# samiazirar/mvtracker

Hardware: AMD Instinct MI355X
Metric: query-points*frames/sec, 4-view 24-frame 512x512 @1024 queries (higher is better)
Workload: dtype bf16; 1 GPU; c3: 4-view synthetic 24-frame 512x512, 1024 queries, bf16 (configs[2], the metric's config); 4-view 24-frame 512x512, 1024 queries per GPU, corr K=16 x 4 levels, iters=4, 3 windows, random-init weights (seeded recipe); queries_total=1024, parallelism=query-shard x1, frame_store=bf16 rows

## Files before the change

### mvtracker_amd/csrc/block_fused.hip

```cpp
#include "common.h"
#include <stdlib.h>

namespace {

typedef __bf16 bf16x8 __attribute__((ext_vector_type(8)));
typedef __bf16 bf16x4 __attribute__((ext_vector_type(4)));
typedef unsigned u32x4 __attribute__((ext_vector_type(4)));
typedef unsigned u32x2 __attribute__((ext_vector_type(2)));

__device__ __forceinline__ void lds_barrier() {
#ifdef MVT_FULL_BARRIERS
  __syncthreads();
#else
  __builtin_amdgcn_fence(__ATOMIC_RELEASE, "workgroup", "local");
  __builtin_amdgcn_s_barrier();
  __builtin_amdgcn_fence(__ATOMIC_ACQUIRE, "workgroup", "local");
#endif
}

constexpr int NT = 512;
constexpr int C = 256;
constexpr int LDX = C + 8;
template <int NMB> struct Cfg {
  static constexpr int BM = 32 * NMB;
// ... 278 lines not shown
                                             int vstride = 0) {
  const int r = lane & 31, h = lane >> 5;
  const float scale = 1.0f / sqrtf((float)DHA);
  auto stage_vt = [&](int kb, unsigned short* img) {
    const int key = kb * 32 + r;
#pragma unroll
    for (int i = 0; i < 6; ++i) {
      u32x2 w = f.v[kb][i];
      if (key >= nk) w = (u32x2){0u, 0u};
#pragma unroll
      for (int e = 0; e < 4; ++e) img[(24 * h + 4 * i + e) * LDVA + r] = (unsigned short)((e & 1) ? (w[e >> 1] >> 16) : (w[e >> 1] & 0xFFFFu));
    }
  };
  if (vstride > 0) {
    __builtin_amdgcn_fence(__ATOMIC_SEQ_CST, "wavefront");
#pragma unroll
    for (int kb = 0; kb < NKB; ++kb) stage_vt(kb, vt + kb * vstride);
    __builtin_amdgcn_fence(__ATOMIC_SEQ_CST, "wavefront");
  }
  __builtin_amdgcn_sched_barrier(0);
  ASTAMP(49);
  bf16x8 qf[NMBQ][3];
#pragma unroll
  for (int mb = 0; mb < NMBQ; ++mb) {
#pragma unroll
    for (int ks = 0; ks < 3; ++ks) {
      f32x4 a = bf4_to_f32(f.q[mb][ks][0], f.q[mb][ks][1]), b = bf4_to_f32(f.q[mb][ks][2], f.q[mb][ks][3]);
#pragma unroll
      for (int e = 0; e < 4; ++e) {
        a[e] *= scale;
        b[e] *= scale;
      }
      const bf16x4 x = __builtin_convertvector(a, bf16x4), y = __builtin_convertvector(b, bf16x4);
#pragma unroll
      for (int e = 0; e < 4; ++e) {
        qf[mb][ks][e] = x[e];
        qf[mb][ks][4 + e] = y[e];
      }
    }
  }
  const unsigned bdm = bd > 0 ? (65536u / (unsigned)bd + 1u) : 0u;
#pragma unroll
  for (int mb = 0; mb < NMBQ; ++mb) {
    const int qi = mb * 32 + r;
    const unsigned qt = ((unsigned)qi * bdm) >> 16;
    f32x16 sc[NKB];
    float mx = -INFINITY;
#pragma unroll
    for (int kb = 0; kb < NKB; ++kb) {
#pragma unroll
      for (int e = 0; e < 16; ++e) sc[kb][e] = 0.f;
#pragma unroll
      for (int ks = 0; ks < 3; ++ks) sc[kb] = __builtin_amdgcn_mfma_f32_32x32x16_bf16(__builtin_bit_cast(bf16x8, f.k[kb][ks]), qf[mb][ks], sc[kb], 0, 0, 0);
    }
#pragma unroll
    for (int kb = 0; kb < NKB; ++kb) {
      const bool half = nk <= kb * 32 + 16;
#pragma unroll
      for (int e = 0; e < 16; ++e) {
        const unsigned kk = (unsigned)(kb * 32 + (e & 3) + 8 * (e >> 2)) + 4u * (unsigned)h;
        const bool ok = (kk < (unsigned)nk) & (((kk * bdm) >> 16) == qt);
        sc[kb][e] = ok ? sc[kb][e] : -INFINITY;
      }
#pragma unroll
      for (int e = 0; e < 8; ++e) mx = fmaxf(mx, sc[kb][e]);
      if (!half) {
#pragma unroll
        for (int e = 8; e < 16; ++e) mx = fmaxf(mx, sc[kb][e]);
      }
    }
    mx = pair_max(mx);
    if (mx == -INFINITY) mx = 0.f;
    float ps = 0.f;
#pragma unroll
    for (int kb = 0; kb < NKB; ++kb) {
      const bool half = nk <= kb * 32 + 16;
#pragma unroll
      for (int e = 0; e < 8; ++e) {
        sc[kb][e] = __expf(sc[kb][e] - mx);
        ps += sc[kb][e];
      }
      if (!half) {
#pragma unroll
        for (int e = 8; e < 16; ++e) {
          sc[kb][e] = __expf(sc[kb][e] - mx);
          ps += sc[kb][e];
        }
      }
    }
    __builtin_amdgcn_sched_barrier(0);
    ASTAMP(50 + 2 * mb);
    f32x16 oacc[2];
#pragma unroll
    for (int db = 0; db < 2; ++db)
#pragma unroll
      for (int e = 0; e < 16; ++e) oacc[db][e] = 0.f;
#pragma unroll
    for (int kb = 0; kb < NKB; ++kb) {
      const bool half = nk <= kb * 32 + 16;
      const unsigned short* vimg = vt + kb * vstride;
      if (vstride == 0 && (mb == 0 || NKB > 1)) {
        __builtin_amdgcn_fence(__ATOMIC_SEQ_CST, "wavefront");
        stage_vt(kb, vt);
        __builtin_amdgcn_fence(__ATOMIC_SEQ_CST, "wavefront");
      }
#pragma unroll
      for (int sk = 0; sk < 2; ++sk) {
        if (sk == 1 && half) break;
        f32x4 lo4, hi4;
#pragma unroll
        for (int e = 0; e < 4; ++e) {
          lo4[e] = sc[kb][8 * sk + e];
          hi4[e] = sc[kb][8 * sk + 4 + e];
        }
        const bf16x4 bl = __builtin_convertvector(lo4, bf16x4), bh = __builtin_convertvector(hi4, bf16x4);
        bf16x8 pb;
#pragma unroll
        for (int e = 0; e < 4; ++e) {
          pb[e] = bl[e];
          pb[4 + e] = bh[e];
        }
#pragma unroll
        for (int db = 0; db < 2; ++db) {
          const unsigned short* vr = (db * 32 + r < DHA) ? &vimg[(db * 32 + r) * LDVA + 16 * sk + 4 * h] : zrow + 16 * sk + 4 * h;
          const u32x2 a0 = *reinterpret_cast<const u32x2*>(vr), a1 = *reinterpret_cast<const u32x2*>(vr + 8);
          const bf16x8 va = __builtin_bit_cast(bf16x8, (u32x4){a0[0], a0[1], a1[0], a1[1]});
          oacc[db] = __builtin_amdgcn_mfma_f32_32x32x16_bf16(va, pb, oacc[db], 0, 0, 0);
        }
      }
    }
    __builtin_amdgcn_sched_barrier(0);
    ASTAMP(51 + 2 * mb);
    const float lt = pair_sum(ps);
    const float inv = 1.0f / lt;
    if (qi >= nq) continue;
#pragma unroll
    for (int db = 0; db < 2; ++db) {
#pragma unroll
      for (int gq = 0; gq < 4; ++gq) {
        const int d = db * 32 + 8 * gq + 4 * h;
        if (d < DHA) {
          f32x4 t;
#pragma unroll
          for (int e = 0; e < 4; ++e) t[e] = oacc[db][4 * gq + e] * inv;
          *reinterpret_cast<u32x2*>(&As[(arow0 + qi) * lda + hd * DHA + d]) = __builtin_bit_cast(u32x2, __builtin_convertvector(t, bf16x4));
        }
      }
    }
  }
}

template <int NMB>
__device__ __forceinline__ void ln_to_lds(const f32x16 (&v)[NMB], unsigned short* Xs, float* st, int wave, int lane, float eps,
                                          const float* lnw, const float* lnb, float (&ms)[NMB][2], bool have) {
  constexpr int BM = 32 * NMB;
  const int r = lane & 31, h = lane >> 5;
  f32x4 gw[4], gb[4];
  if (lnw) {
#pragma unroll
    for (int g = 0; g < 4; ++g) {
      gw[g] = *reinterpret_cast<const f32x4*>(lnw + wave * 32 + 8 * g + 4 * h);
      gb[g] = *reinterpret_cast<const f32x4*>(lnb + wave * 32 + 8 * g + 4 * h);
    }
  }
  if (!have) {
#pragma unroll
    for (int mb = 0; mb < NMB; ++mb) {
      float s1 = 0.f, s2 = 0.f;
#pragma unroll
      for (int e = 0; e < 16; ++e) {
        s1 += v[mb][e];
        s2 = fmaf(v[mb][e], v[mb][e], s2);
      }
      s1 += __shfl_xor(s1, 32, 64);
      s2 += __shfl_xor(s2, 32, 64);
      if (h == 0) {
        st[(wave * BM + mb * 32 + r) * 2] = s1;
        st[(wave * BM + mb * 32 + r) * 2 + 1] = s2;
      }
    }
    lds_barrier();
#pragma unroll
    for (int mb = 0; mb < NMB; ++mb) {
      float s1 = 0.f, s2 = 0.f;
#pragma unroll
      for (int w = 0; w < 8; ++w) {
        s1 += st[(w * BM + mb * 32 + r) * 2];
        s2 += st[(w * BM + mb * 32 + r) * 2 + 1];
      }
      const float mean = s1 / (float)C;
      ms[mb][0] = mean;
      ms[mb][1] = fmaxf(s2 / (float)C - mean * mean, 0.f);
    }
  }
#pragma unroll
  for (int mb = 0; mb < NMB; ++mb) {
    const float mean = ms[mb][0];
    const float rstd = 1.0f / sqrtf(ms[mb][1] + eps);
#pragma unroll
    for (int g = 0; g < 4; ++g) {
      const int n = wave * 32 + 8 * g + 4 * h;
      f32x4 o;
#pragma unroll
      for (int e = 0; e < 4; ++e) {
        o[e] = (v[mb][4 * g + e] - mean) * rstd;
        if (lnw) o[e] = o[e] * gw[g][e] + gb[g][e];
      }
      const bf16x4 b = __builtin_convertvector(o, bf16x4);
      *reinterpret_cast<u32x2*>(&Xs[(mb * 32 + r) * LDX + n]) = __builtin_bit_cast(u32x2, b);
    }
  }
  lds_barrier();
}

template <int NMB, int MODE, int ATT>
__global__ __launch_bounds__(NT) void block_fused_bf16(BlockArgs p) {
  using K_ = Cfg<NMB>;
  constexpr int BM = K_::BM, HC = K_::HC, LDH = K_::LDH, LDA = K_::LDA;
  constexpr bool CTX = ATT == 6;
  static_assert(!CTX || (NMB == 2 && MODE == 0), "ATT 6 runs on the 64-row tiles of the point rows");
  constexpr int HSZ = CTX && (64 * LDKV + 1) / 2 > BM * LDH ? (64 * LDKV + 1) / 2 : BM * LDH;
  __shared__ __attribute__((aligned(16))) unsigned short Xs[BM * LDX];
  __shared__ __attribute__((aligned(16))) unsigned short Hs[2][HSZ];
  __shared__ float st[8 * BM * 2];
  __shared__ __attribute__((aligned(16))) float b1s[4 * C];
  __shared__ __attribute__((aligned(16))) float cbs[CTX ? 2 * 288 : 4];

  const int t = threadIdx.x, wave = t >> 6, lane = t & 63;
  const int r = lane & 31, h = lane >> 5;
  int bx = (int)blockIdx.x, by = (int)blockIdx.y, bz = (int)blockIdx.z;
  if constexpr (ATT == 2 || ATT == 3 || ATT == 5 || ATT == 6) {
    const unsigned total = gridDim.x * gridDim.y * gridDim.z;
    if (total % 8 == 0) {
      const unsigned L = blockIdx.x + gridDim.x * (blockIdx.y + gridDim.y * blockIdx.z);
      const unsigned V = (L % 8) * (total / 8) + L / 8;
      bx = (int)(V % gridDim.x);
      by = (int)((V / gridDim.x) % gridDim.y);
      bz = (int)(V / (gridDim.x * gridDim.y));
    }
  }
  static_assert(ATT == 0 || ATT == 5 || MODE != 2, "pass 2 of the split path has no attention");
  static_assert(ATT != 5 || MODE == 2, "ATT 5 = pass 2 on the frame-major tiles of an ATT 2 / ATT 3 pass 1");
  static_assert((MODE != 1 && MODE != 2) || NMB == 1, "the split path runs on 32-row tiles");
  constexpr bool FM = ATT == 2 || ATT == 3 || ATT == 5 || ATT == 6;
  const int bmv = ATT == 1 ? p.bmv : BM;
  const long long m0 = FM ? 0 : (long long)bx * bmv;
  const long long ntok = FM ? p.M / p.S : 0;
  auto grow = [&](int i) -> long long {
    if (FM) {
      const long long tk = (long long)bx * BM + i;
      return tk < ntok ? tk * p.S + (long long)bz : -1;
    }
    const long long m = m0 + i;
    return (i < bmv && m < p.M) ? m : -1;
  };
  const long long rlo = FM ? (long long)bx * BM * p.S : m0;
  const long long rhi = FM ? ((long long)bx * BM + BM) * p.S : m0 + bmv;
  constexpr bool HAS_MLP = MODE == 0 || MODE == 1;
  if (HAS_MLP)
    for (int i = t; i < p.H; i += NT) b1s[i] = p.b1[i];
  const long long ws_tile = FM ? (long long)bz * gridDim.x + bx : (long long)bx;
  const long long ws_ntile = FM ? (long long)gridDim.z * gridDim.x : (long long)gridDim.x;
  auto ws_off = [&](int chunk, int g) -> long long { return ((((long long)chunk * ws_ntile + ws_tile) * 8 + wave) * 4 + g) * 256 + lane * 4; };
  auto active = [&](int q) { return q < p.n_next && rlo < p.next[q].row_hi && rhi > p.next[q].row_lo; };
  bf16x8 wq[PFQ];
  constexpr bool EARLY = NMB == 1 && MODE != 0;
  bool early_have = false;
  const bool outp = MODE != 2 && ATT != 4 && (ATT != 0 || p.att != nullptr);
  const unsigned short* wo_row = p.wo + ((long long)wave * 18 * 64 + lane) * 8;
  const unsigned short* fc1_first = p.w1 + ((long long)(wave % K_::JW) * (C / 16) * 64 + lane) * 8 +
                                    (long long)(MODE == 1 ? by : 0) * K_::JW * (C / 16) * FS;
  auto prefetch_wo = [&]() { fill_wq(wq, wo_row); };
  if (HAS_MLP && !outp) {
    fill_wq(wq, fc1_first);
  } else if (CTX) {
    fill_wq(wq, p.c_kv.w + ((long long)wave * (C / 16) * 64 + lane) * 8);
  } else if (outp) {
    prefetch_wo();
  } else if (EARLY && MODE == 2) {
    const int nb0e = by * 8 + wave;
    if (active(0) && nb0e < (p.next[0].N + 31) / 32) {
      fill_wq(wq, p.next[0].w + ((long long)nb0e * (C / 16) * 64 + lane) * 8);
      early_have = true;
    }
  }

  STAMP(0);
  f32x16 v[NMB];
#pragma unroll
  for (int mb = 0; mb < NMB; ++mb)
#pragma unroll
    for (int e = 0; e < 16; ++e) v[mb][e] = 0.f;

  f32x4 xr[NMB][4];
  auto load_x = [&]() {
    if (ATT == 4 || (MODE == 2 && p.ws)) return;
#pragma unroll
    for (int mb = 0; mb < NMB; ++mb) {
      const long long m = grow(mb * 32 + r);
#pragma unroll
      for (int g = 0; g < 4; ++g)
        xr[mb][g] = m >= 0 ? *reinterpret_cast<const f32x4*>(p.x + m * (long long)p.ldx + wave * 32 + 8 * g + 4 * h) : (f32x4){0.f, 0.f, 0.f, 0.f};
    }
  };

  bf16x8 wx[2];
  auto pre_gemm = [&]() {
    wx[0] = ldg_frag(wo_row + 16 * FS);
    wx[1] = ldg_frag(wo_row + 17 * FS);
    load_x();
  };

  if constexpr (CTX) {
    constexpr int KVB = 2 * 288 / 32;
    unsigned short* KV = &Hs[0][0];
    unsigned short* XN = &Xs[0];
    for (int i = t; i < KVB * 32; i += NT) cbs[i] = p.c_kv.b[i];
    const long long ctile = 2LL * gridDim.z;
    auto cws_off = [&](int chunk, int mb, int g) -> long long {
      return ((((long long)chunk * ctile + (long long)bz * 2 + mb) * 8 + wave) * 4 + g) * 256 + lane * 4;
    };
    constexpr int MAXCH = 4;
    const int nch = p.c_nch;
    f32x16 cv[2];
#pragma unroll
    for (int gh = 0; gh < 2; ++gh) {
      f32x4 part[2][2][MAXCH + 1], b2v[2];
#pragma unroll
      for (int mb = 0; mb < 2; ++mb)
#pragma unroll
        for (int g = 0; g < 2; ++g)
#pragma unroll
          for (int sidx = 0; sidx <= MAXCH; ++sidx)
            part[mb][g][sidx] = sidx <= nch ? *reinterpret_cast<const f32x4*>(p.c_ws + cws_off(sidx, mb, 2 * gh + g)) : (f32x4){0.f, 0.f, 0.f, 0.f};
#pragma unroll
      for (int g = 0; g < 2; ++g) b2v[g] = *reinterpret_cast<const f32x4*>(p.c_b2 + wave * 32 + 8 * (2 * gh + g) + 4 * h);
      __builtin_amdgcn_sched_barrier(0);
#pragma unroll
      for (int mb = 0; mb < 2; ++mb)
#pragma unroll
        for (int g = 0; g < 2; ++g) {
          f32x4 xv = part[mb][g][0];
#pragma unroll
          for (int sidx = 1; sidx <= MAXCH; ++sidx)
            if (sidx <= nch) {
#pragma unroll
              for (int e = 0; e < 4; ++e) xv[e] += part[mb][g][sidx][e];
            }
#pragma unroll
          for (int e = 0; e < 4; ++e) cv[mb][4 * (2 * gh + g) + e] = 0.f + (xv[e] + b2v[g][e]);
        }
      __builtin_amdgcn_sched_barrier(0);
    }
    STAMP(56);
    auto krow_w = [&](int nb) { return p.c_kv.w + ((long long)nb * (C / 16) * 64 + lane) * 8; };
    auto nrow_w = [&](int nb) { return p.c_next.w + ((long long)nb * (C / 16) * 64 + lane) * 8; };
    if (bx == 0) {
#pragma unroll
      for (int mb = 0; mb < 2; ++mb) {
        const long long m = (long long)(mb * 32 + r) * p.S + (long long)bz;
#pragma unroll
        for (int g = 0; g < 4; ++g) {
          f32x4 o;
#pragma unroll
          for (int e = 0; e < 4; ++e) o[e] = cv[mb][4 * g + e];
          *reinterpret_cast<f32x4*>(p.c_x + m * (long long)p.c_ldx + wave * 32 + 8 * g + 4 * h) = o;
        }
      }
    }
    float cms[2][2];
    ln_to_lds<2>(cv, XN, st, wave, lane, p.c_kv.eps, p.c_kv.lnw, p.c_kv.lnb, cms, false);
    STAMP(57);
    const int nnb = p.c_next.w ? (p.c_next.N + 31) / 32 : 0;
    const bool do_next = bx * 8 < nnb;
    const int nbn = bx * 8 + wave;
    const bool my_next = nbn < nnb;
#pragma unroll 1
    for (int nb = wave; nb < KVB; nb += 8) {
// ... 278 lines not shown
    STAMP(2);
    lds_barrier();
    STAMP(3);
    gemm_wq18<NMB, HAS_MLP>(v, wq, wx, fc1_first, &As[r * LDA + 8 * h], LDA);
#pragma unroll
    for (int mb = 0; mb < NMB; ++mb)
#pragma unroll
      for (int e = 0; e < 16; ++e) v[mb][e] += p.bo[wave * 32 + (e & 3) + 8 * (e >> 2) + 4 * h];
  } else {
    load_x();
  }
  STAMP(4);
  if (MODE == 2 && p.ws) {
    constexpr int MAXCH = 4;
    const int nch = p.H / Cfg<NMB>::HC;
    f32x4 part[NMB][4][MAXCH + 1];
#pragma unroll
    for (int mb = 0; mb < NMB; ++mb) {
      const long long m = grow(mb * 32 + r);
#pragma unroll
      for (int g = 0; g < 4; ++g)
#pragma unroll
        for (int sidx = 0; sidx <= MAXCH; ++sidx)
          part[mb][g][sidx] = (m >= 0 && sidx <= nch) ? *reinterpret_cast<const f32x4*>(p.ws + ws_off(sidx, g)) : (f32x4){0.f, 0.f, 0.f, 0.f};
    }
    __builtin_amdgcn_sched_barrier(0);
#pragma unroll
    for (int mb = 0; mb < NMB; ++mb)
#pragma unroll
      for (int g = 0; g < 4; ++g) {
        f32x4 xv = part[mb][g][0];
#pragma unroll
        for (int sidx = 1; sidx <= MAXCH; ++sidx)
          if (sidx <= nch) {
#pragma unroll
            for (int e = 0; e < 4; ++e) xv[e] += part[mb][g][sidx][e];
          }
#pragma unroll
        for (int e = 0; e < 4; ++e) v[mb][4 * g + e] += xv[e] + p.b2[wave * 32 + 8 * g + 4 * h + e];
      }
  } else if (ATT != 4) {
#pragma unroll
    for (int mb = 0; mb < NMB; ++mb)
#pragma unroll
      for (int g = 0; g < 4; ++g)
#pragma unroll
        for (int e = 0; e < 4; ++e) v[mb][4 * g + e] += xr[mb][g][e];
  }

  auto store_x = [&]() {
#pragma unroll
    for (int mb = 0; mb < NMB; ++mb) {
      const long long m = grow(mb * 32 + r);
      if (m >= 0) {
#pragma unroll
        for (int g = 0; g < 4; ++g) {
          f32x4 o;
#pragma unroll
          for (int e = 0; e < 4; ++e) o[e] = v[mb][4 * g + e];
          *reinterpret_cast<f32x4*>(p.x + m * (long long)p.ldx + wave * 32 + 8 * g + 4 * h) = o;
        }
      }
    }
  };
  STAMP(5);
  float ln_ms[NMB][2];
  if (HAS_MLP) ln_to_lds<NMB>(v, Xs, st, wave, lane, 1e-6f, nullptr, nullptr, ln_ms, false);
  STAMP(6);
  const bool tail_next = MODE == 0 && active(0) && wave < (p.next[0].N + 31) / 32;
  if (HAS_MLP) {
    f32x16 acc2[NMB];
#pragma unroll
    for (int mb = 0; mb < NMB; ++mb)
#pragma unroll
      for (int e = 0; e < 16; ++e) acc2[mb][e] = 0.f;
    constexpr int JW = K_::JW, NM1 = K_::NM1;
    const int jb = wave % JW, mp = wave / JW;
    const int nchunk = p.H / HC;
    const unsigned short* w1row = p.w1 + ((long long)jb * (C / 16) * 64 + lane) * 8;
    const unsigned short* w2row = p.w2 + ((long long)wave * (p.H / 16) * 64 + lane) * 8;
    static_assert(HC / 16 == PFQ && C / 16 == PFQ, "every GEMM segment is exactly one queue length");
    const unsigned short* tail = tail_next ? p.next[0].w + ((long long)wave * (C / 16) * 64 + lane) * 8 : w1row;
    const int c_lo = MODE == 1 ? by : 0, c_hi = MODE == 1 ? c_lo + 1 : nchunk;
#pragma unroll 1
    for (int c = c_lo; c < c_hi; ++c) {
      unsigned short* Hb = Hs[c & 1];
      f32x16 ha[NM1];
#pragma unroll
      for (int i = 0; i < NM1; ++i)
#pragma unroll
        for (int e = 0; e < 16; ++e) ha[i][e] = 0.f;
      STAMP(8 + 5 * c);
      gemm_wq<C / 16, NM1>(ha, wq, w1row + (long long)c * JW * (C / 16) * FS, w2row + (long long)c * (HC / 16) * FS, &Xs[r * LDX + 8 * h], LDX,
                           NM1 * mp);
      STAMP(9 + 5 * c);
#pragma unroll
      for (int i = 0; i < NM1; ++i) {
#pragma unroll
        for (int g = 0; g < 4; ++g) {
          const f32x4 bq = *reinterpret_cast<const f32x4*>(&b1s[c * HC + jb * 32 + 8 * g + 4 * h]);
          f32x4 o;
#ifdef MVT_ABL_NOGELU
#pragma unroll
          for (int e = 0; e < 4; ++e) o[e] = ha[i][4 * g + e] + bq[e];
#else
#pragma unroll
          for (int e = 0; e < 4; e += 2) {
            const f32x2 y = gelu_tanh_pk((f32x2){ha[i][4 * g + e] + bq[e], ha[i][4 * g + e + 1] + bq[e + 1]});
            o[e] = y[0];
            o[e + 1] = y[1];
          }
#endif
          const bf16x4 b = __builtin_convertvector(o, bf16x4);
          *reinterpret_cast<u32x2*>(&Hb[((NM1 * mp + i) * 32 + r) * LDH + jb * 32 + 8 * g + 4 * h]) = __builtin_bit_cast(u32x2, b);
        }
      }
      STAMP(10 + 5 * c);
      lds_barrier();
      STAMP(11 + 5 * c);
      const unsigned short* after = c + 1 < c_hi ? w1row + (long long)(c + 1) * JW * (C / 16) * FS : tail;
      gemm_wq<HC / 16, NMB>(acc2, wq, w2row + (long long)c * (HC / 16) * FS, after, &Hb[r * LDH + 8 * h], LDH, 0);
      STAMP(12 + 5 * c);
    }
    if (MODE == 1) {
#pragma unroll
      for (int mb = 0; mb < NMB; ++mb) {
        const long long m = grow(mb * 32 + r);
        if (m < 0) continue;
#pragma unroll
        for (int g = 0; g < 4; ++g) {
          f32x4 a4, x4;
#pragma unroll
          for (int e = 0; e < 4; ++e) {
            a4[e] = acc2[mb][4 * g + e];
            x4[e] = v[mb][4 * g + e];
          }
          *reinterpret_cast<f32x4*>(p.ws + ws_off(by + 1, g)) = a4;
          if (by == 0) *reinterpret_cast<f32x4*>(p.ws + ws_off(0, g)) = x4;
        }
      }
      return;
    }
#pragma unroll
    for (int mb = 0; mb < NMB; ++mb)
#pragma unroll
      for (int g = 0; g < 4; ++g)
#pragma unroll
        for (int e = 0; e < 4; ++e) v[mb][4 * g + e] += acc2[mb][4 * g + e] + p.b2[wave * 32 + 8 * g + 4 * h + e];
  }
  STAMP(30);
  if (MODE == 0 || ATT == 4 || (p.ws && by == 0)) store_x();
  STAMP(31);

  bool have = tail_next || early_have;
  bool have_ms = false;
#pragma unroll
  for (int q = 0; q < MVT_BLOCK_MAX_NEXT; ++q) {
    if (q >= p.n_next) break;
    if (!active(q)) continue;
    const mvt_block_next nx = p.next[q];
    lds_barrier();
    for (int i = t; i < nx.N; i += NT) b1s[i] = nx.b[i];
    STAMP(32 + 8 * q);
    ln_to_lds<NMB>(v, Xs, st, wave, lane, nx.eps, nx.lnw, nx.lnb, ln_ms, have_ms);
    have_ms = true;
    STAMP(33 + 8 * q);
    const int nblocks = (nx.N + 31) / 32;
    auto nrow_of = [&](int nb) { return nx.w + ((long long)nb * (C / 16) * 64 + lane) * 8; };
    const int nb0 = MODE == 2 ? by * 8 + wave : wave, nbstep = MODE == 2 ? 8 * (int)gridDim.y : 8;
    if (nb0 < nblocks && !have) fill_wq(wq, nrow_of(nb0));
    const int qn = q + 1 < MVT_BLOCK_MAX_NEXT ? q + 1 : MVT_BLOCK_MAX_NEXT - 1;
    const unsigned short* chain = nullptr;
    if ((MODE == 0 || MODE == 3) && q + 1 < MVT_BLOCK_MAX_NEXT && active(q + 1) && wave < (p.next[qn].N + 31) / 32)
      chain = p.next[qn].w + ((long long)wave * (C / 16) * 64 + lane) * 8;
    have = chain != nullptr && wave < nblocks;
    for (int nb = nb0; nb < nblocks; nb += nbstep) {
      f32x16 acc[NMB];
#pragma unroll
      for (int mb = 0; mb < NMB; ++mb)
#pragma unroll
        for (int e = 0; e < 16; ++e) acc[mb][e] = 0.f;
      gemm_wq<C / 16, NMB>(acc, wq, nrow_of(nb), nb + nbstep < nblocks ? nrow_of(nb + nbstep) : (chain ? chain : nrow_of(nb)), &Xs[r * LDX + 8 * h], LDX, 0);
      STAMP(34 + 8 * q + (nb - nb0) / nbstep);
      if (nx.y_bf16 && nb * 32 + 31 < nx.N && (nx.ldy & 7) == 0 && ((uintptr_t)nx.y & 15) == 0) {
        unsigned short* tile = &Hs[0][0] + wave * (NMB * 32 * YLD);
        __builtin_amdgcn_fence(__ATOMIC_SEQ_CST, "wavefront");
#pragma unroll
        for (int mb = 0; mb < NMB; ++mb)
#pragma unroll
          for (int g = 0; g < 4; ++g) {
            f32x4 o;
#pragma unroll
            for (int e = 0; e < 4; ++e) o[e] = acc[mb][4 * g + e] + b1s[nb * 32 + 8 * g + 4 * h + e];
            *reinterpret_cast<u32x2*>(&tile[(mb * 32 + r) * YLD + 8 * g + 4 * h]) = __builtin_bit_cast(u32x2, __builtin_convertvector(o, bf16x4));
          }
        __builtin_amdgcn_fence(__ATOMIC_SEQ_CST, "wavefront");
        unsigned short* yb = reinterpret_cast<unsigned short*>(nx.y) + nb * 32;
#pragma unroll
        for (int k = 0; k < NMB * 2; ++k) {
          const int pc = lane + 64 * k, row = pc >> 2, c = pc & 3;
          const long long m = grow(row);
          if (m >= nx.row_lo && m < nx.row_hi)
            *reinterpret_cast<u32x4*>(yb + m * (long long)nx.ldy + c * 8) = *reinterpret_cast<const u32x4*>(&tile[row * YLD + c * 8]);
        }
        continue;
      }
#pragma unroll
      for (int mb = 0; mb < NMB; ++mb) {
        const long long m = grow(mb * 32 + r);
        if (m < nx.row_lo || m >= nx.row_hi) continue;
#pragma unroll
        for (int g = 0; g < 4; ++g) {
          const int n = nb * 32 + 8 * g + 4 * h;
          if (n + 3 < nx.N) {
            f32x4 o;
#pragma unroll
            for (int e = 0; e < 4; ++e) o[e] = acc[mb][4 * g + e] + b1s[n + e];
            store_act4(nx.y, m * (long long)nx.ldy + n, o, nx.y_bf16);
          } else {
#pragma unroll
            for (int e = 0; e < 4; ++e)
              if (n + e < nx.N) store_act(nx.y, m * (long long)nx.ldy + n + e, acc[mb][4 * g + e] + b1s[n + e], nx.y_bf16);
          }
        }
      }
    }
    STAMP(39 + 8 * q);
  }
  STAMP(63);
}

__global__ void pack_frag_kernel(const unsigned short* __restrict__ w, int ld, int N, int K, unsigned short* __restrict__ out) {
  const long long total = (long long)((N + 31) / 32) * (K / 16) * 64;
  for (long long i = blockIdx.x * (long long)blockDim.x + threadIdx.x; i < total; i += (long long)gridDim.x * blockDim.x) {
    const int lane = (int)(i & 63);
    const long long f = i >> 6;
    const int ks = (int)(f % (K / 16));
    const int nb = (int)(f / (K / 16));
    const int n = nb * 32 + (lane & 31), k = ks * 16 + 8 * (lane >> 5);
    u32x4 v = (u32x4){0u, 0u, 0u, 0u};
    if (n < N) v = *reinterpret_cast<const u32x4*>(w + (long long)n * ld + k);
    *reinterpret_cast<u32x4*>(out + i * 8) = v;
  }
}

}

#ifdef MVT_STAMPS
extern "C" int mvt_debug_read_stamps(unsigned long long* host) {
  return hipMemcpyFromSymbol(host, HIP_SYMBOL(mvt_stamp_buf), sizeof(unsigned long long) * 2 * 8 * 64) == hipSuccess ? MVT_OK : MVT_ERR_HIP_BASE;
}
extern "C" int mvt_debug_clear_stamps() {
  static unsigned long long z[2 * 8 * 64];
  return hipMemcpyToSymbol(HIP_SYMBOL(mvt_stamp_buf), z, sizeof(z)) == hipSuccess ? MVT_OK : MVT_ERR_HIP_BASE;
}
#endif

extern "C" int mvt_pack_frag_bf16(const unsigned short* w, int ld, int N, int K, unsigned short* out, void* stream) {
  MVT_REQUIRE(w && out && N > 0 && K > 0 && K % 16 == 0 && ld % 8 == 0 && ld >= K);
  MVT_REQUIRE(((uintptr_t)w % 16 == 0) && ((uintptr_t)out % 16 == 0));
  const long long total = (long long)((N + 31) / 32) * (K / 16) * 64;
  hipLaunchKernelGGL(pack_frag_kernel, dim3((unsigned)mvt_cdiv(total, 256)), dim3(256), 0, mvt_stream(stream), w, ld, N, K, out);
  return mvt_launch_status();
}

extern "C" int mvt_block_fused_bf16(float* x, int ldx, const void* att, int att_bf16, int ldatt, int Ko, const unsigned short* wo, int ldwo,
                                    const float* bo, const unsigned short* w1, int ldw1, const float* b1, const unsigned short* w2,
                                    int ldw2, const float* b2, int H, const mvt_block_next* next, int n_next, long long M, int Cc,
                                    float* workspace, void* stream) {
  MVT_REQUIRE(x && w1 && b1 && w2 && b2 && M > 0 && Cc == C && H > 0 && H % 256 == 0 && H <= 4 * C);
  MVT_REQUIRE(ldx % 4 == 0 && ldx >= C);
  MVT_REQUIRE(!att || (wo && bo && Ko == 288 && ldatt % 4 == 0 && ldatt >= Ko));
  MVT_REQUIRE(n_next >= 0 && n_next <= MVT_BLOCK_MAX_NEXT && (n_next == 0 || next));
  MVT_REQUIRE(((uintptr_t)x % 16 == 0) && ((uintptr_t)att % 16 == 0) && ((uintptr_t)wo % 16 == 0) && ((uintptr_t)w1 % 16 == 0) &&
              ((uintptr_t)w2 % 16 == 0));
  BlockArgs a{};
  a.x = x; a.ldx = ldx; a.att = (const float*)att; a.att_bf16 = att_bf16 ? 1 : 0; a.ldatt = ldatt; a.Ko = Ko; a.wo = wo; a.bo = bo; a.ldwo = ldwo;
  a.w1 = w1; a.b1 = b1; a.w2 = w2; a.b2 = b2; a.ldw1 = ldw1; a.ldw2 = ldw2; a.H = H; a.M = M; a.n_next = n_next;
  for (int q = 0; q < n_next; ++q) {
    const mvt_block_next& nx = next[q];
    MVT_REQUIRE(nx.w && nx.b && nx.y && nx.N > 0 && nx.N <= 4 * C && nx.ldy % 4 == 0 && nx.ldy >= nx.N);
    MVT_REQUIRE(nx.y_bf16 == 0 || nx.y_bf16 == 1);
    MVT_REQUIRE((nx.lnw == nullptr) == (nx.lnb == nullptr) && ((uintptr_t)nx.lnw % 16 == 0) && ((uintptr_t)nx.lnb % 16 == 0) && ((uintptr_t)nx.w % 16 == 0) && ((uintptr_t)nx.y % 16 == 0));
    MVT_REQUIRE(nx.row_lo >= 0 && (nx.row_hi == 0 || nx.row_hi > nx.row_lo));
    a.next[q] = nx;
    if (nx.row_hi == 0) a.next[q].row_hi = M;
  }
  static const char* force = getenv("MVT_BLOCK_NMB");
  const int nmb = force ? atoi(force) : (M >= 4096 ? 2 : 1);
  static const bool no_split = getenv("MVT_BLOCK_NOSPLIT") != nullptr;
  a.ws = workspace;
  if (nmb == 2) {
    hipLaunchKernelGGL((block_fused_bf16<2, 0, 0>), dim3((unsigned)mvt_cdiv(M, 64)), dim3(NT), 0, mvt_stream(stream), a);
  } else if (workspace && !no_split && M <= 2048 && M % 32 == 0) {
    MVT_REQUIRE((uintptr_t)workspace % 16 == 0);
    const unsigned tiles = (unsigned)mvt_cdiv(M, 32);
    hipLaunchKernelGGL((block_fused_bf16<1, 1, 0>), dim3(tiles, (unsigned)(H / 256)), dim3(NT), 0, mvt_stream(stream), a);
    int maxblk = 1;
    for (int q = 0; q < n_next; ++q) maxblk = (next[q].N + 31) / 32 > maxblk ? (next[q].N + 31) / 32 : maxblk;
    const unsigned slices = n_next ? (unsigned)mvt_cdiv(maxblk, 8) : 1u;
    hipLaunchKernelGGL((block_fused_bf16<1, 2, 0>), dim3(tiles, slices), dim3(NT), 0, mvt_stream(stream), a);
  } else {
    hipLaunchKernelGGL((block_fused_bf16<1, 0, 0>), dim3((unsigned)mvt_cdiv(M, 32)), dim3(NT), 0, mvt_stream(stream), a);
  }
  return mvt_launch_status();
}

extern "C" int mvt_attn_block_fused_bf16(float* x, int ldx, const mvt_block_attn* attn, const unsigned short* wo, const float* bo,
                                         const unsigned short* w1, const float* b1, const unsigned short* w2, const float* b2, int H,
                                         const mvt_block_next* next, int n_next, long long M, int Cc, float* workspace, void* stream) {
  MVT_REQUIRE(x && attn && wo && bo && w1 && b1 && w2 && b2 && M > 0 && Cc == C && H > 0 && H % 256 == 0 && H <= 4 * C);
  MVT_REQUIRE(ldx % 4 == 0 && ldx >= C && n_next >= 0 && n_next <= MVT_BLOCK_MAX_NEXT && (n_next == 0 || next));
  MVT_REQUIRE(attn->heads == 6 && attn->dim_head == DHA && attn->S >= 1 && M % attn->S == 0);
  MVT_REQUIRE(attn->kind == MVT_ATTN_PARTIALS || (attn->kind == MVT_ATTN_FRAME_CTX && attn->q && attn->ldq % 8 == 0 && attn->ldq >= 288) ||
              (attn->q && attn->k && attn->v && attn->ldq % 8 == 0 && attn->ldkv % 8 == 0 && attn->ldq >= 288 && attn->ldkv >= 288));
  MVT_REQUIRE(((uintptr_t)x % 16 == 0) && ((uintptr_t)wo % 16 == 0) && ((uintptr_t)w1 % 16 == 0) && ((uintptr_t)w2 % 16 == 0));
  MVT_REQUIRE(((uintptr_t)attn->q % 16 == 0) && ((uintptr_t)attn->k % 16 == 0) && ((uintptr_t)attn->v % 16 == 0));
  BlockArgs a{};
  a.x = x; a.ldx = ldx; a.att = nullptr; a.Ko = 288; a.wo = wo; a.bo = bo; a.ldwo = 288;
  a.w1 = w1; a.b1 = b1; a.w2 = w2; a.b2 = b2; a.ldw1 = C; a.ldw2 = H; a.H = H; a.M = M; a.n_next = n_next; a.ws = workspace;
  a.aq = attn->q; a.ak = attn->k; a.av = attn->v; a.ldaq = attn->ldq; a.ldakv = attn->ldkv; a.S = attn->S; a.nkeys = attn->n_keys;
  for (int q = 0; q < n_next; ++q) {
    const mvt_block_next& nx = next[q];
    MVT_REQUIRE(nx.w && nx.b && nx.y && nx.N > 0 && nx.N <= 4 * C && nx.ldy % 4 == 0 && nx.ldy >= nx.N);
    MVT_REQUIRE((nx.y_bf16 == 0 || nx.y_bf16 == 1) && (nx.lnw == nullptr) == (nx.lnb == nullptr) && ((uintptr_t)nx.lnw % 16 == 0) && ((uintptr_t)nx.lnb % 16 == 0));
    MVT_REQUIRE(((uintptr_t)nx.w % 16 == 0) && ((uintptr_t)nx.y % 16 == 0) && nx.row_lo >= 0 && (nx.row_hi == 0 || nx.row_hi > nx.row_lo));
    a.next[q] = nx;
    if (nx.row_hi == 0) a.next[q].row_hi = M;
  }
  const int S = attn->S;
  if (attn->kind == MVT_ATTN_TIME) {
    MVT_REQUIRE(S <= 32 && !workspace);
    static const bool small_tiles = !(getenv("MVT_TIME_NMB1") && atoi(getenv("MVT_TIME_NMB1")) == 0);
    if (small_tiles && mvt_cdiv(M, (32 / S) * S) <= 256) {
      a.bmv = (32 / S) * S;
      hipLaunchKernelGGL((block_fused_bf16<1, 0, 1>), dim3((unsigned)mvt_cdiv(M, a.bmv)), dim3(NT), 0, mvt_stream(stream), a);
      return mvt_launch_status();
    }
    a.bmv = (64 / S) * S;
    hipLaunchKernelGGL((block_fused_bf16<2, 0, 1>), dim3((unsigned)mvt_cdiv(M, a.bmv)), dim3(NT), 0, mvt_stream(stream), a);
  } else if (attn->kind == MVT_ATTN_PARTIALS) {
    MVT_REQUIRE(attn->partials && attn->n_splits >= 1 && attn->n_splits <= MVT_ATTN_NSPLIT && attn->n_keys == 64 && M == 64LL * S);
    MVT_REQUIRE(workspace && (uintptr_t)workspace % 16 == 0 && M <= 2048 && (uintptr_t)attn->partials % 16 == 0);
    a.parts = attn->partials; a.nsplit = attn->n_splits;
    const unsigned tiles = (unsigned)mvt_cdiv(M, 32);
    a.S = S;
    hipLaunchKernelGGL((block_fused_bf16<1, 1, 3>), dim3(2, (unsigned)(H / 256), (unsigned)S), dim3(NT), 0, mvt_stream(stream), a);
    int maxblk = 1;
    for (int q = 0; q < n_next; ++q) maxblk = (next[q].N + 31) / 32 > maxblk ? (next[q].N + 31) / 32 : maxblk;
    const unsigned slices = n_next ? (unsigned)mvt_cdiv(maxblk, 8) : 1u;
    (void)tiles;
    if (!attn->defer_pass2)
      hipLaunchKernelGGL((block_fused_bf16<1, 2, 5>), dim3(2, slices, (unsigned)S), dim3(NT), 0, mvt_stream(stream), a);
  } else if (attn->kind == MVT_ATTN_FRAME) {
    MVT_REQUIRE(attn->n_keys >= 1 && attn->n_keys <= 64);
    const long long ntok = M / S;
    static const bool small_tiles = !(getenv("MVT_FRAME_NMB1") && atoi(getenv("MVT_FRAME_NMB1")) == 0);
    if (ntok * S >= 4096 && small_tiles && mvt_cdiv(ntok, 32) * S <= 256) {
      MVT_REQUIRE(!workspace);
      hipLaunchKernelGGL((block_fused_bf16<1, 0, 2>), dim3((unsigned)mvt_cdiv(ntok, 32), 1, (unsigned)S), dim3(NT), 0, mvt_stream(stream), a);
    } else if (ntok * S >= 4096) {
      MVT_REQUIRE(!workspace);
      hipLaunchKernelGGL((block_fused_bf16<2, 0, 2>), dim3((unsigned)mvt_cdiv(ntok, 64), 1, (unsigned)S), dim3(NT), 0, mvt_stream(stream), a);
    } else {
      MVT_REQUIRE(workspace && (uintptr_t)workspace % 16 == 0 && M <= 2048 && ntok % 32 == 0);
      hipLaunchKernelGGL((block_fused_bf16<1, 1, 2>), dim3((unsigned)(ntok / 32), (unsigned)(H / 256), (unsigned)S), dim3(NT), 0,
                         mvt_stream(stream), a);
      int maxblk = 1;
      for (int q = 0; q < n_next; ++q) maxblk = (next[q].N + 31) / 32 > maxblk ? (next[q].N + 31) / 32 : maxblk;
      const unsigned slices = n_next ? (unsigned)mvt_cdiv(maxblk, 8) : 1u;
      if (!attn->defer_pass2)
        hipLaunchKernelGGL((block_fused_bf16<1, 2, 5>), dim3((unsigned)(ntok / 32), slices, (unsigned)S), dim3(NT), 0, mvt_stream(stream), a);
    }
  } else if (attn->kind == MVT_ATTN_FRAME_CTX) {
    const mvt_block_ctx* cx = attn->ctx;
    const long long ntok = M / S;
    MVT_REQUIRE(cx && attn->n_keys == 64 && ntok * S >= 4096 && !workspace && !attn->defer_pass2);
    MVT_REQUIRE(cx->ws && cx->b2 && cx->x && cx->chunks >= 1 && cx->chunks <= 4 && cx->ldx % 4 == 0 && cx->ldx >= C);
    MVT_REQUIRE(((uintptr_t)cx->ws % 16 == 0) && ((uintptr_t)cx->b2 % 16 == 0) && ((uintptr_t)cx->x % 16 == 0));
    MVT_REQUIRE(cx->kv.w && cx->kv.b && cx->kv.N == 2 * 288 && (cx->kv.lnw == nullptr) == (cx->kv.lnb == nullptr));
// ... 87 lines not shown
```

Baseline: 1.005 million query-points*frames/s.

## Merge trailing next-layer GEMMs into grouped column loops sharing normalized LDS tiles

The tail of the fused block kernel used to run each follow-on projection (next[q]) as its own loop: a barrier, a bias load, a LayerNorm write into LDS, then column blocks spread over the 8 waves. This change packs consecutive projections into groups. Each group has one combined column-block index space, a shared bias buffer, and up to two normalized activation buffers (a second LDS tile when ATT==1), and projections with the same LN parameters reuse one buffer. The aim is fewer barriers and better wave balance when a single projection has too few column blocks for all waves. The costs are extra LDS, runtime selection of the projection per column block, and loss of the cross-projection weight prefetch chain.

```diff
diff --git a/mvtracker_amd/csrc/block_fused.hip b/mvtracker_amd/csrc/block_fused.hip
--- a/mvtracker_amd/csrc/block_fused.hip
+++ b/mvtracker_amd/csrc/block_fused.hip
@@ -454,7 +454,7 @@
 
 template <int NMB>
 __device__ __forceinline__ void ln_to_lds(const f32x16 (&v)[NMB], unsigned short* Xs, float* st, int wave, int lane, float eps,
-                                          const float* lnw, const float* lnb, float (&ms)[NMB][2], bool have) {
+                                          const float* lnw, const float* lnb, float (&ms)[NMB][2], bool have, bool sync = true) {
   constexpr int BM = 32 * NMB;
   const int r = lane & 31, h = lane >> 5;
   f32x4 gw[4], gb[4];
@@ -512,7 +512,7 @@
       *reinterpret_cast<u32x2*>(&Xs[(mb * 32 + r) * LDX + n]) = __builtin_bit_cast(u32x2, b);
     }
   }
-  lds_barrier();
+  if (sync) lds_barrier();
 }
 
 template <int NMB, int MODE, int ATT>
@@ -522,10 +522,13 @@
   constexpr bool CTX = ATT == 6;
   static_assert(!CTX || (NMB == 2 && MODE == 0), "ATT 6 runs on the 64-row tiles of the point rows");
   constexpr int HSZ = CTX && (64 * LDKV + 1) / 2 > BM * LDH ? (64 * LDKV + 1) / 2 : BM * LDH;
+  constexpr int NA = ATT == 1 ? 2 : 1;
+  constexpr int BCAP = ATT == 1 ? 6 * C : 4 * C;
   __shared__ __attribute__((aligned(16))) unsigned short Xs[BM * LDX];
+  __shared__ __attribute__((aligned(16))) unsigned short Xn2[NA > 1 ? BM * LDX : 8];
   __shared__ __attribute__((aligned(16))) unsigned short Hs[2][HSZ];
   __shared__ float st[8 * BM * 2];
-  __shared__ __attribute__((aligned(16))) float b1s[4 * C];
+  __shared__ __attribute__((aligned(16))) float b1s[BCAP];
   __shared__ __attribute__((aligned(16))) float cbs[CTX ? 2 * 288 : 4];
 
   const int t = threadIdx.x, wave = t >> 6, lane = t & 63;
@@ -1110,37 +1113,106 @@
   if (MODE == 0 || ATT == 4 || (p.ws && by == 0)) store_x();
   STAMP(31);
 
+  int grp[MVT_BLOCK_MAX_NEXT], abuf[MVT_BLOCK_MAX_NEXT], boff[MVT_BLOCK_MAX_NEXT], nbk[MVT_BLOCK_MAX_NEXT];
+  int ngrp = 0;
+  {
+    int nbuf = 0, bfill = 0;
+#pragma unroll
+    for (int q = 0; q < MVT_BLOCK_MAX_NEXT; ++q) {
+      grp[q] = -1;
+      abuf[q] = 0;
+      boff[q] = 0;
+      nbk[q] = 0;
+      if (!active(q)) continue;
+      const int N = p.next[q].N;
+      nbk[q] = (N + 31) / 32;
+      int share = -1;
+#pragma unroll
+      for (int q2 = 0; q2 < q; ++q2)
+        if (ngrp > 0 && grp[q2] == ngrp - 1 && p.next[q2].eps == p.next[q].eps && p.next[q2].lnw == p.next[q].lnw &&
+            p.next[q2].lnb == p.next[q].lnb)
+          share = abuf[q2];
+      if (ngrp == 0 || (share < 0 && nbuf == NA) || bfill + N > BCAP) {
+        ++ngrp;
+        nbuf = 0;
+        bfill = 0;
+        share = -1;
+      }
+      grp[q] = ngrp - 1;
+      abuf[q] = share >= 0 ? share : nbuf++;
+      boff[q] = bfill;
+      bfill += N;
+    }
+  }
   bool have = tail_next || early_have;
   bool have_ms = false;
-#pragma unroll
-  for (int q = 0; q < MVT_BLOCK_MAX_NEXT; ++q) {
-    if (q >= p.n_next) break;
-    if (!active(q)) continue;
-    const mvt_block_next nx = p.next[q];
+  const int j0 = __builtin_amdgcn_readfirstlane(MODE == 2 ? by * 8 + wave : wave), jstep = MODE == 2 ? 8 * (int)gridDim.y : 8;
+#pragma unroll 1
+  for (int G = 0; G < ngrp; ++G) {
+    int s0[MVT_BLOCK_MAX_NEXT], T = 0, nvar = 0;
+#pragma unroll
+    for (int q = 0; q < MVT_BLOCK_MAX_NEXT; ++q) {
+      s0[q] = T;
+      if (grp[q] == G) {
+        T += nbk[q];
+        nvar = abuf[q] + 1 > nvar ? abuf[q] + 1 : nvar;
+      }
+    }
     lds_barrier();
-    for (int i = t; i < nx.N; i += NT) b1s[i] = nx.b[i];
-    STAMP(32 + 8 * q);
-    ln_to_lds<NMB>(v, Xs, st, wave, lane, nx.eps, nx.lnw, nx.lnb, ln_ms, have_ms);
-    have_ms = true;
-    STAMP(33 + 8 * q);
-    const int nblocks = (nx.N + 31) / 32;
-    auto nrow_of = [&](int nb) { return nx.w + ((long long)nb * (C / 16) * 64 + lane) * 8; };
-    const int nb0 = MODE == 2 ? by * 8 + wave : wave, nbstep = MODE == 2 ? 8 * (int)gridDim.y : 8;
-    if (nb0 < nblocks && !have) fill_wq(wq, nrow_of(nb0));
-    const int qn = q + 1 < MVT_BLOCK_MAX_NEXT ? q + 1 : MVT_BLOCK_MAX_NEXT - 1;
-    const unsigned short* chain = nullptr;
-    if ((MODE == 0 || MODE == 3) && q + 1 < MVT_BLOCK_MAX_NEXT && active(q + 1) && wave < (p.next[qn].N + 31) / 32)
-      chain = p.next[qn].w + ((long long)wave * (C / 16) * 64 + lane) * 8;
-    have = chain != nullptr && wave < nblocks;
-    for (int nb = nb0; nb < nblocks; nb += nbstep) {
+#pragma unroll
+    for (int q = 0; q < MVT_BLOCK_MAX_NEXT; ++q)
+      if (grp[q] == G)
+        for (int i = t; i < p.next[q].N; i += NT) b1s[boff[q] + i] = p.next[q].b[i];
+    STAMP(32 + 8 * G);
+#pragma unroll
+    for (int a = 0; a < NA; ++a) {
+      if (a >= nvar) break;
+      int qa = 0;
+#pragma unroll
+      for (int q = MVT_BLOCK_MAX_NEXT - 1; q >= 0; --q)
+        if (grp[q] == G && abuf[q] == a) qa = q;
+      const float eps = qa == 0 ? p.next[0].eps : qa == 1 ? p.next[1].eps : p.next[2].eps;
+      const float* lnw = qa == 0 ? p.next[0].lnw : qa == 1 ? p.next[1].lnw : p.next[2].lnw;
+      const float* lnb = qa == 0 ? p.next[0].lnb : qa == 1 ? p.next[1].lnb : p.next[2].lnb;
+      ln_to_lds<NMB>(v, a ? Xn2 : Xs, st, wave, lane, eps, lnw, lnb, ln_ms, have_ms, a + 1 == nvar);
+      have_ms = true;
+    }
+    STAMP(33 + 8 * G);
+    auto qof = [&](int j) {
+      int qq = 0;
+#pragma unroll
+      for (int q = 0; q < MVT_BLOCK_MAX_NEXT; ++q)
+        if (grp[q] == G && j >= s0[q]) qq = q;
+      return qq;
+    };
+    auto wrow_of = [&](int j) {
+      const int q = qof(j);
+      const unsigned short* w = q == 0 ? p.next[0].w : q == 1 ? p.next[1].w : p.next[2].w;
+      return w + ((long long)(j - s0[q]) * (C / 16) * 64 + lane) * 8;
+    };
+    if (j0 < T && !have) fill_wq(wq, wrow_of(j0));
+    have = false;
+    for (int j = j0; j < T; j += jstep) {
+      const int q = qof(j), nb = j - s0[q];
+      const mvt_block_next& n0 = p.next[0];
+      const mvt_block_next& n1 = p.next[1];
+      const mvt_block_next& n2 = p.next[2];
+      float* const ny = q == 0 ? n0.y : q == 1 ? n1.y : n2.y;
+      const int nN = q == 0 ? n0.N : q == 1 ? n1.N : n2.N;
+      const int nldy = q == 0 ? n0.ldy : q == 1 ? n1.ldy : n2.ldy;
+      const int ny_bf16 = q == 0 ? n0.y_bf16 : q == 1 ? n1.y_bf16 : n2.y_bf16;
+      const long long nlo = q == 0 ? n0.row_lo : q == 1 ? n1.row_lo : n2.row_lo;
+      const long long nhi = q == 0 ? n0.row_hi : q == 1 ? n1.row_hi : n2.row_hi;
+      const float* bq = &b1s[q == 0 ? boff[0] : q == 1 ? boff[1] : boff[2]];
+      const unsigned short* As = (q == 0 ? abuf[0] : q == 1 ? abuf[1] : abuf[2]) ? Xn2 : Xs;
       f32x16 acc[NMB];
 #pragma unroll
       for (int mb = 0; mb < NMB; ++mb)
 #pragma unroll
         for (int e = 0; e < 16; ++e) acc[mb][e] = 0.f;
-      gemm_wq<C / 16, NMB>(acc, wq, nrow_of(nb), nb + nbstep < nblocks ? nrow_of(nb + nbstep) : (chain ? chain : nrow_of(nb)), &Xs[r * LDX + 8 * h], LDX, 0);
-      STAMP(34 + 8 * q + (nb - nb0) / nbstep);
-      if (nx.y_bf16 && nb * 32 + 31 < nx.N && (nx.ldy & 7) == 0 && ((uintptr_t)nx.y & 15) == 0) {
+      gemm_wq<C / 16, NMB>(acc, wq, wrow_of(j), j + jstep < T ? wrow_of(j + jstep) : wrow_of(j), &As[r * LDX + 8 * h], LDX, 0);
+      STAMP(34 + 8 * G + ((j - j0) / jstep < 4 ? (j - j0) / jstep : 4));
+      if (ny_bf16 && nb * 32 + 31 < nN && (nldy & 7) == 0 && ((uintptr_t)ny & 15) == 0) {
         unsigned short* tile = &Hs[0][0] + wave * (NMB * 32 * YLD);
         __builtin_amdgcn_fence(__ATOMIC_SEQ_CST, "wavefront");
 #pragma unroll
@@ -1149,41 +1221,41 @@
           for (int g = 0; g < 4; ++g) {
             f32x4 o;
 #pragma unroll
-            for (int e = 0; e < 4; ++e) o[e] = acc[mb][4 * g + e] + b1s[nb * 32 + 8 * g + 4 * h + e];
+            for (int e = 0; e < 4; ++e) o[e] = acc[mb][4 * g + e] + bq[nb * 32 + 8 * g + 4 * h + e];
             *reinterpret_cast<u32x2*>(&tile[(mb * 32 + r) * YLD + 8 * g + 4 * h]) = __builtin_bit_cast(u32x2, __builtin_convertvector(o, bf16x4));
           }
         __builtin_amdgcn_fence(__ATOMIC_SEQ_CST, "wavefront");
-        unsigned short* yb = reinterpret_cast<unsigned short*>(nx.y) + nb * 32;
+        unsigned short* yb = reinterpret_cast<unsigned short*>(ny) + nb * 32;
 #pragma unroll
         for (int k = 0; k < NMB * 2; ++k) {
           const int pc = lane + 64 * k, row = pc >> 2, c = pc & 3;
           const long long m = grow(row);
-          if (m >= nx.row_lo && m < nx.row_hi)
-            *reinterpret_cast<u32x4*>(yb + m * (long long)nx.ldy + c * 8) = *reinterpret_cast<const u32x4*>(&tile[row * YLD + c * 8]);
+          if (m >= nlo && m < nhi)
+            *reinterpret_cast<u32x4*>(yb + m * (long long)nldy + c * 8) = *reinterpret_cast<const u32x4*>(&tile[row * YLD + c * 8]);
         }
         continue;
       }
 #pragma unroll
       for (int mb = 0; mb < NMB; ++mb) {
         const long long m = grow(mb * 32 + r);
-        if (m < nx.row_lo || m >= nx.row_hi) continue;
+        if (m < nlo || m >= nhi) continue;
 #pragma unroll
         for (int g = 0; g < 4; ++g) {
           const int n = nb * 32 + 8 * g + 4 * h;
-          if (n + 3 < nx.N) {
+          if (n + 3 < nN) {
             f32x4 o;
 #pragma unroll
-            for (int e = 0; e < 4; ++e) o[e] = acc[mb][4 * g + e] + b1s[n + e];
-            store_act4(nx.y, m * (long long)nx.ldy + n, o, nx.y_bf16);
+            for (int e = 0; e < 4; ++e) o[e] = acc[mb][4 * g + e] + bq[n + e];
+            store_act4(ny, m * (long long)nldy + n, o, ny_bf16);
           } else {
 #pragma unroll
             for (int e = 0; e < 4; ++e)
-              if (n + e < nx.N) store_act(nx.y, m * (long long)nx.ldy + n + e, acc[mb][4 * g + e] + b1s[n + e], nx.y_bf16);
+              if (n + e < nN) store_act(ny, m * (long long)nldy + n + e, acc[mb][4 * g + e] + bq[n + e], ny_bf16);
           }
         }
       }
     }
-    STAMP(39 + 8 * q);
+    STAMP(39 + 8 * G);
   }
   STAMP(63);
 }
```

Result: no change. 1.013 million query-points*frames/s, median of 6 (+0.8%).
